# tangjiapeng/DiffuScene

Measured on AMD Instinct MI355X. Metric: denoiser steps/sec (train + 1000-step sample) at B=256, N=80 objects, higher is better.
Workload: dtype f32 (operands split 3xbf16, 6 products, f32 accumulate); 1 GPU; uncond living/dining rooms (config/uncond/diffusion_livingrooms_instancond_lat32_v.yaml scaled to N=80), B=256 scenes per GPU, N=80, C=65, T=1000, mode=both; global_batch=256, parallelism=single

## Files before the change

### __graft_entry__.py

```python
import os
import subprocess
import sys

ROOT = os.path.dirname(os.path.abspath(__file__))
CSRC = os.path.join(ROOT, "diffuscene_amd", "csrc")
LIB = os.path.join(ROOT, "diffuscene_amd", "libdiffuscene_hip.so")

SOURCES = [
    ("gemm_mfma.hip", []),
    ("gemm_split.hip", ["-fno-slp-vectorize"]),
    ("gemm_tn_split.hip", ["-fno-slp-vectorize"]),
    ("blocks.hip", []),
    ("diffusion.hip", ["-ffp-contract=off"]),
    ("train.hip", []),
    ("retrieval.hip", ["-ffp-contract=off"]),
    ("dataset.hip", ["-ffp-contract=off"]),
    ("chamfer.hip", ["-ffp-contract=off"]),
    ("optim.hip", ["-ffp-contract=off"]),
    ("foldingnet.hip", []),
]


def _hipcc():
    for c in (os.environ.get("HIPCC"), "/opt/rocm/bin/hipcc", "hipcc"):
        if c and (os.path.isabs(c) and os.path.exists(c) or not os.path.isabs(c)):
            return c
    raise RuntimeError("hipcc not found")


def _stale(target, deps):
    if not os.path.exists(target):
        return True
    t = os.path.getmtime(target)
    return any(os.path.getmtime(d) > t for d in deps)


def _stamp_git_head():
    try:
        head = subprocess.check_output(["git", "rev-parse", "--short", "HEAD"], cwd=ROOT, stderr=subprocess.DEVNULL, text=True).strip()
        dirty = subprocess.check_output(["git", "status", "--porcelain", "-uno"], cwd=ROOT, stderr=subprocess.DEVNULL, text=True).strip()
        with open(os.path.join(ROOT, "GIT_HEAD"), "w") as f:
            f.write(head + ("+" if dirty else "") + "\n")
    except Exception:
        pass

# ... 95 lines not shown
```

### diffuscene_amd/_lib.py

```python
import ctypes as C
import os

_HERE = os.path.dirname(os.path.abspath(__file__))
LIB_PATH = os.path.join(_HERE, "libdiffuscene_hip.so")
if os.environ.get("DSC_HIP_LIB"):
    LIB_PATH = os.path.abspath(os.environ["DSC_HIP_LIB"])

ACT_NONE, ACT_GELU, ACT_SILU, ACT_LEAKY01 = 0, 1, 2, 3
SS_NONE, SS_PER_TOKEN, SS_PER_SCENE, SS_PER_SLOT, SS_BY_INDEX = 0, 1, 2, 3, 4
MEAN_EPS, MEAN_X0, MEAN_V = 0, 1, 2
TILE_GN_80_W8, TILE_GN_80_W4, TILE_160x256, TILE_160x128_W4 = 1, 2, 5, 8
TILE_WAVE_GN, TILE_WAVE_DENSE, TILE_WAVE_GN_64 = 10, 11, 12
F32_TILE_160x256, F32_TILE_160x128, F32_TILE_128x128, F32_TILE_96x128, F32_TILE_64x64 = 0, 1, 2, 3, 4
DSC_PLANES_NONE = -100
GEMM_ROW_INVARIANT = 1
WS_MAX = 64
MAX_TOKENS_PER_SCENE = 160
STATS_MAX_OBJECTS, STATS_ONE_WAVE_MAX = 160, 32

_ERR = {-1: "DSC_EINVAL (bad shape / null pointer)", -2: "DSC_EALIGN (16-byte alignment required)",
        -3: "DSC_ERANGE (size outside kernel limits)"}

c_f32p = C.c_void_p
c_i64p = C.c_void_p


class GemmArgs(C.Structure):
    _fields_ = [
        ("a1", C.c_void_p), ("lda1", C.c_int64), ("k1", C.c_int32),
        ("a2", C.c_void_p), ("lda2", C.c_int64), ("k2", C.c_int32),
        ("w", C.c_void_p), ("ldw", C.c_int64),
        ("bias", C.c_void_p),
        ("residual", C.c_void_p), ("ldr", C.c_int64),
        ("y", C.c_void_p), ("ldy", C.c_int64),
        ("m", C.c_int32), ("n", C.c_int32),
        ("act_in", C.c_int32), ("act_out", C.c_int32),
        ("batch", C.c_int32),
        ("sa1", C.c_int64), ("sa2", C.c_int64), ("sw", C.c_int64), ("sbias", C.c_int64),
        ("sres", C.c_int64), ("sy", C.c_int64),
        ("gamma", C.c_void_p), ("beta", C.c_void_p), ("eps", C.c_float),
        ("tokens_per_scene", C.c_int32),
        ("scale_shift", C.c_void_p), ("ld_ss", C.c_int64), ("ss_mode", C.c_int32),
        ("preact", C.c_void_p), ("ld_preact", C.c_int64),
        ("ss_index", C.c_void_p),
        ("w_planes", C.c_void_p),
        ("actgrad_x", C.c_void_p), ("ld_actgrad", C.c_int64),
        ("ss_rows", C.c_int32),
        ("w_planes_layout", C.c_int32),
        ("gnb_z", C.c_void_p), ("ld_gnb_z", C.c_int64),
        ("gnb_dgamma", C.c_void_p), ("gnb_dbeta", C.c_void_p), ("gnb_dbias", C.c_void_p), ("gnb_pstride", C.c_int64),
        ("gnb_dss", C.c_void_p), ("ld_gnb_dss", C.c_int64),
        ("flags", C.c_int32),
    ]


class SplitItem(C.Structure):
    _fields_ = [("w", C.c_void_p), ("ldw", C.c_int64), ("rows", C.c_int32), ("cols", C.c_int32), ("planes", C.c_void_p),
                ("transpose", C.c_int32)]


class SmallKItem(C.Structure):
    _fields_ = [("x", C.c_void_p), ("ldx", C.c_int64), ("k_in", C.c_int32), ("w", C.c_void_p), ("ldw", C.c_int64), ("bias", C.c_void_p),
                ("y", C.c_void_p), ("ldy", C.c_int64)]


class ColSpan(C.Structure):
    _fields_ = [("src_col", C.c_int32), ("dst_col", C.c_int32), ("width", C.c_int32)]


SMALLK_MAX = 4


class WsItem(C.Structure):
    _fields_ = [("w", C.c_void_p), ("out", C.c_void_p), ("rows", C.c_int32), ("cols", C.c_int32)]


class TnGroup(C.Structure):
    _fields_ = [("a1", C.c_void_p), ("lda1", C.c_int64), ("k1", C.c_int32),
                ("a2", C.c_void_p), ("lda2", C.c_int64), ("k2", C.c_int32),
                ("dy", C.c_void_p), ("ldd", C.c_int64),
                ("out", C.c_void_p), ("ldo", C.c_int64),
                ("dbias", C.c_void_p),
                ("m", C.c_int32), ("n", C.c_int32), ("kvalid", C.c_int32),
                ("tile0", C.c_int32),
                ("ws_offset", C.c_int64),
                ("tile0s", C.c_int32)]


class ColsumItem(C.Structure):
    _fields_ = [("x", C.c_void_p), ("ldx", C.c_int64), ("m", C.c_int32), ("n", C.c_int32), ("out", C.c_void_p)]


class WsBwdItem(C.Structure):
    _fields_ = [("w", C.c_void_p), ("dw_std", C.c_void_p), ("dw", C.c_void_p), ("rows", C.c_int32), ("cols", C.c_int32)]


SIGNATURES = {
    "dsc_version": (C.c_int, []),
    "dsc_gemm_f32": (C.c_int, [C.POINTER(GemmArgs), C.c_void_p]),
    "dsc_gemm_gn_silu_f32": (C.c_int, [C.POINTER(GemmArgs), C.c_void_p]),
    "dsc_split_bf16x3_f32": (C.c_int, [C.POINTER(SplitItem), C.c_int32, C.c_void_p]),
    "dsc_gemm_arithmetic": (C.c_int, [C.POINTER(GemmArgs), C.c_int32]),
    "dsc_gemm_split_tile": (C.c_int, [C.POINTER(GemmArgs), C.c_int32]),
    "dsc_gemm_f32_tile": (C.c_int, [C.POINTER(GemmArgs)]),
    "dsc_gemm_planes_layout": (C.c_int, [C.POINTER(GemmArgs), C.c_int32]),
    "dsc_get_split_wave": (C.c_int, []),
    "dsc_set_split_wave": (C.c_int, [C.c_int32]),
    "dsc_gemm_skinny": (C.c_int, [C.POINTER(GemmArgs), C.c_int32]),
    "dsc_get_skinny": (C.c_int, []),
    "dsc_set_skinny": (C.c_int, [C.c_int32]),
    "dsc_get_gemm_arithmetic": (C.c_int, []),
    "dsc_set_gemm_arithmetic": (C.c_int, [C.c_int32]),
    "dsc_gemm_layernorm_f32": (C.c_int, [C.POINTER(GemmArgs), C.c_void_p]),
    "dsc_gemm_splitk_f32": (C.c_int, [C.POINTER(GemmArgs), C.c_int32, c_f32p, C.c_int64, C.c_void_p]),
    "dsc_linear_smallk_f32": (C.c_int, [c_f32p, C.c_int64, C.c_int32, c_f32p, C.c_int64, c_f32p, c_f32p, C.c_int64,
                                        C.c_int32, C.c_int32, C.c_int32, C.c_void_p]),
    "dsc_linear_smallk_grouped_f32": (C.c_int, [C.POINTER(SmallKItem), C.c_int32, C.c_int32, C.c_int32, C.c_int32, C.c_void_p]),
    "dsc_gather_columns_f32": (C.c_int, [c_f32p, C.c_int64, c_f32p, C.c_int64, C.c_int32, C.POINTER(ColSpan), C.c_int32, C.c_void_p]),
    "dsc_weight_standardize_f32": (C.c_int, [C.POINTER(WsItem), C.c_int32, C.c_float, C.c_void_p]),
    "dsc_layernorm_f32": (C.c_int, [c_f32p, C.c_int64, c_f32p, c_f32p, C.c_int64, c_f32p, C.c_int64, C.c_int32,
                                    C.c_int32, C.c_float, C.c_void_p]),
    "dsc_linear_attention_f32": (C.c_int, [c_f32p, C.c_int64, c_f32p, C.c_int64, c_f32p, C.c_int64, c_f32p, C.c_int64,
                                           C.c_int32, C.c_int32, C.c_int32, C.c_float, C.c_void_p]),
    "dsc_attention_f32": (C.c_int, [c_f32p, C.c_int64, c_f32p, C.c_int64, c_f32p, C.c_int64, c_f32p, C.c_int64,
                                    C.c_int32, C.c_int32, C.c_float, C.c_void_p]),
    "dsc_time_embedding_f32": (C.c_int, [c_i64p, C.c_int32, C.c_int32, c_f32p, C.c_int32, c_f32p, c_f32p, C.c_void_p]),
    "dsc_activation_f32": (C.c_int, [c_f32p, c_f32p, C.c_int64, C.c_int32, C.c_void_p]),
    "dsc_q_sample_f32": (C.c_int, [c_f32p, c_f32p, c_i64p, c_f32p, c_f32p, c_f32p, c_f32p, C.c_int32, C.c_int64, C.c_int32,
                                   C.c_void_p]),
    "dsc_p_sample_f32": (C.c_int, [c_f32p, c_f32p, c_f32p, c_i64p, c_f32p, c_f32p, c_f32p, c_f32p, c_f32p, c_f32p,
                                   c_f32p, C.c_int32, C.c_int32, C.c_int32, C.c_int64, C.c_int32, C.c_void_p]),
    "dsc_device_error_count": (C.c_int64, [C.c_int32]),
    "dsc_add_scalar_i64": (C.c_int, [c_i64p, C.c_int32, C.c_int64, C.c_void_p]),
    "dsc_ddim_step_f32": (C.c_int, [c_f32p, c_f32p, c_f32p, c_i64p, c_i64p, c_i64p, c_f32p, c_f32p, c_f32p, c_f32p, c_f32p,
                                    c_f32p, c_f32p, c_f32p, c_f32p, C.c_int32, C.c_int32, C.c_int64, C.c_int32, C.c_int32,
                                    C.c_void_p]),
    "dsc_ddim_advance_i64": (C.c_int, [c_i64p, c_i64p, c_i64p, C.c_int32, C.c_int32, C.c_void_p]),
    "dsc_knn16_f32": (C.c_int, [c_f32p, C.c_int64, C.c_int32, c_f32p, c_f32p, C.c_int32, C.c_int32, C.c_void_p, C.c_void_p]),
    "dsc_rowsq_f32": (C.c_int, [c_f32p, C.c_int64, C.c_int32, C.c_int64, c_f32p, C.c_void_p]),
    "dsc_knn_cov_f32": (C.c_int, [c_f32p, C.c_int64, C.c_void_p, C.c_int32, C.c_int32, c_f32p, C.c_int64, C.c_void_p]),
    "dsc_gather_max_f32": (C.c_int, [c_f32p, C.c_int64, C.c_void_p, C.c_int32, C.c_int32, C.c_int32, c_f32p, C.c_int64,
                                     C.c_void_p, C.c_void_p]),
    "dsc_gather_max_bwd_f32": (C.c_int, [c_f32p, C.c_int64, C.c_void_p, C.c_void_p, C.c_int32, C.c_int32, C.c_int32, c_f32p,
                                         C.c_int64, C.c_void_p]),
    "dsc_bn_workspace_floats": (C.c_int64, [C.c_int64, C.c_int32]),
    "dsc_batchnorm_fwd_f32": (C.c_int, [c_f32p, C.c_int64, c_f32p, c_f32p, C.c_int64, C.c_int32, C.c_float, C.c_float,
# ... 99 lines not shown
def load():
    global _lib
    if _lib is not None:
        return _lib
    if not os.path.exists(LIB_PATH):
        raise HipLibraryMissing(
            "%s not found: build it with `python __graft_entry__.py` (hipcc --offload-arch=gfx950). "
            "diffuscene_amd has no CPU or PyTorch fallback." % LIB_PATH)
    import torch
    lib = C.CDLL(LIB_PATH)
    for name, (res, args) in SIGNATURES.items():
        try:
            fn = getattr(lib, name)
        except AttributeError as e:
            raise HipLibraryMissing("symbol %s missing from %s" % (name, LIB_PATH)) from e
        fn.restype = res
        fn.argtypes = args
    if lib.dsc_get_gemm_arithmetic() < 0:
        raise ValueError("DSC_GEMM=%r: must be 'split' (default) or 'f32'" % os.environ.get("DSC_GEMM"))
    if lib.dsc_get_tn_split_form() < 0:
        raise ValueError("DSC_TN_FORM=%r: must be '2' (default), '1' or '0'" % os.environ.get("DSC_TN_FORM"))
    if lib.dsc_get_split_wave() < 0:
        raise ValueError("DSC_WAVE=%r: must be '1' / 'auto' (default) or '0'" % os.environ.get("DSC_WAVE"))
    _lib = lib
    return lib


def split_enabled():
    return load().dsc_get_gemm_arithmetic() == 1


def gemm_mode():
    lib = load()
    if lib.dsc_get_gemm_arithmetic() != 1:
        return 0
    return (2 if lib.dsc_get_split_wave() == 1 else 1) + 10 * lib.dsc_get_tn_split_form()


def set_split_wave(on):
    prev = load().dsc_get_split_wave() == 1
    check(load().dsc_set_split_wave(1 if on else 0), "dsc_set_split_wave")
    return prev


def set_gemm_arithmetic(name):
    if name not in ("split", "f32"):
        raise ValueError("gemm arithmetic must be 'split' or 'f32', got %r" % (name,))
    prev = "split" if split_enabled() else "f32"
    check(load().dsc_set_gemm_arithmetic(1 if name == "split" else 0), "dsc_set_gemm_arithmetic")
    return prev


def device_error_count(reset=False):
    n = load().dsc_device_error_count(1 if reset else 0)
    if n < 0:
        raise RuntimeError("dsc_device_error_count failed (HIP error)")
    return int(n)


def check_indices(where):
    if os.environ.get("DSC_CHECK_INDICES", "0") == "1":
        n = device_error_count(reset=True)
        if n:
            raise IndexError("%s: %d out-of-range device timestep(s) were clamped into the schedule tables" % (where, n))


def check(rc, what):
    if rc != 0:
        raise RuntimeError("%s failed: %s" % (what, _ERR.get(rc, "hipError_t %d" % rc)))
# ... 5 lines not shown
```

### diffuscene_amd/csrc/dsc_common.h

```cpp
#pragma once
#include <hip/hip_runtime.h>
#include <stdint.h>
#include <type_traits>
#include "../../include/diffuscene_hip.h"

typedef float f32x2 __attribute__((ext_vector_type(2)));
typedef float f32x4 __attribute__((ext_vector_type(4)));
typedef float f32x16 __attribute__((ext_vector_type(16)));

#define DSC_WAVE 64

#include <utility>
template <class F, int... I>
__device__ __forceinline__ void dsc_static_for_impl(F&& f, std::integer_sequence<int, I...>) { (f(std::integral_constant<int, I>{}), ...); }
template <int N, class F>
__device__ __forceinline__ void dsc_static_for(F&& f) { dsc_static_for_impl(f, std::make_integer_sequence<int, N>{}); }

#define DSC_CLEAR_STALE_ERROR() ((void)hipGetLastError())

#define DSC_LAUNCH_CHECK()                                   \
    do {                                                     \
        hipError_t e__ = hipGetLastError();                  \
        if (e__ != hipSuccess) return (int)e__;              \
    } while (0)
// ... 44 lines not shown
    const int waves = (n + 15) / 16;
    return waves >= 8 ? 512u : 64u * (unsigned)waves;
}

__device__ __forceinline__ float wave_sum(float v) {
#pragma unroll
    for (int o = 32; o > 0; o >>= 1) v += __shfl_xor(v, o, 64);
    return v;
}
__device__ __forceinline__ float wave_sum_dpp(float v) {
    auto dpp_add = [](float x, auto ctrl, auto row_mask, auto bank_mask) {
        const int y = __builtin_amdgcn_update_dpp(0, __builtin_bit_cast(int, x), decltype(ctrl)::value, decltype(row_mask)::value,
                                                  decltype(bank_mask)::value, true);
        return x + __builtin_bit_cast(float, y);
    };
    using std::integral_constant;
    v = dpp_add(v, integral_constant<int, 0x111>{}, integral_constant<int, 0xf>{}, integral_constant<int, 0xf>{});
    v = dpp_add(v, integral_constant<int, 0x112>{}, integral_constant<int, 0xf>{}, integral_constant<int, 0xf>{});
    v = dpp_add(v, integral_constant<int, 0x114>{}, integral_constant<int, 0xf>{}, integral_constant<int, 0xf>{});
    v = dpp_add(v, integral_constant<int, 0x118>{}, integral_constant<int, 0xf>{}, integral_constant<int, 0xf>{});
    v = dpp_add(v, integral_constant<int, 0x142>{}, integral_constant<int, 0xa>{}, integral_constant<int, 0xf>{});
    v = dpp_add(v, integral_constant<int, 0x143>{}, integral_constant<int, 0xc>{}, integral_constant<int, 0xf>{});
    return __builtin_bit_cast(float, __builtin_amdgcn_readlane(__builtin_bit_cast(int, v), 63));
}
__device__ __forceinline__ float wave_max(float v) {
#pragma unroll
    for (int o = 32; o > 0; o >>= 1) v = fmaxf(v, __shfl_xor(v, o, 64));
    return v;
}

#define DSC_SPLIT_NOT_TAKEN (-1000)
int dsc_gemm_try_split(const dsc_gemm_args* a, bool gn, hipStream_t s);

int dsc_launch_reduce_grouped(const dsc_tn_group* groups_dev, int count, int total_tiles, int splits, const float* workspace, hipStream_t s);

#ifdef DSC_BAD_INDEX_COUNTER
static __device__ unsigned int dsc_bad_index_count = 0;
__device__ __forceinline__ int64_t dsc_checked_index(int64_t v, int64_t n, bool first = true) {
    if (v < 0 || v >= n) {
        if (first) atomicAdd(&dsc_bad_index_count, 1u);
        return (v < 0 || n < 1) ? 0 : n - 1;
    }
    return v;
}
static inline unsigned dsc_read_bad_index_count(bool reset) {
    unsigned v = 0;
    if (hipMemcpyFromSymbol(&v, HIP_SYMBOL(dsc_bad_index_count), sizeof(v)) != hipSuccess) return 0xffffffffu;
    if (reset && v) {
        const unsigned z = 0;
        (void)hipMemcpyToSymbol(HIP_SYMBOL(dsc_bad_index_count), &z, sizeof(z));
    }
    return v;
}
#endif
unsigned dsc_bad_index_diffusion(bool reset);
unsigned dsc_bad_index_train(bool reset);
unsigned dsc_bad_index_retrieval(bool reset);
__device__ __forceinline__ int64_t dsc_clamp_index(int64_t v, int64_t n) { return (v < 0 || n < 1) ? 0 : (v >= n ? n - 1 : v); }

static inline bool dsc_aligned16(const void* p) { return (reinterpret_cast<uintptr_t>(p) & 15u) == 0; }
```

### diffuscene_amd/csrc/gemm_mfma.hip

```cpp
#include "gemm_core.h"
#include "gemm_skinny.h"
#include <cstdlib>

namespace {

using dsc_gemm::gemm_kernel;
constexpr int BK = 32;

int check_common(const dsc_gemm_args* a) {
    if (!a || !a->a1 || !a->w || !a->y) return DSC_EINVAL;
    if (a->m <= 0 || a->n <= 0 || a->k1 <= 0 || a->k2 < 0) return DSC_EINVAL;
    if ((a->k1 % BK) || (a->k2 % BK)) return DSC_EINVAL;
    if (a->k2 > 0 && !a->a2) return DSC_EINVAL;
    if (a->batch < 1) return DSC_EINVAL;
    if (!dsc_aligned16(a->a1) || (a->lda1 & 3) || !dsc_aligned16(a->w) || (a->ldw & 3)) return DSC_EALIGN;
    if (a->k2 > 0 && (!dsc_aligned16(a->a2) || (a->lda2 & 3))) return DSC_EALIGN;
    if (a->batch > 1 && ((a->sa1 & 3) || (a->sa2 & 3) || (a->sw & 3))) return DSC_EALIGN;
    if (a->act_in != DSC_ACT_NONE) return DSC_EINVAL;
    if (a->act_out < DSC_ACT_NONE || a->act_out > DSC_ACT_SILU) return DSC_EINVAL;
    return 0;
}

template <int TM, int TN, int WM, int WN, bool GN, int IL>
int launch_il(const dsc_gemm_args* a, int rows_per_blk, hipStream_t s) {
// ... 212 lines not shown
        default: return launch<1, 1, 2, 2, true, 0>(a, rpb, s);
    }
}

extern "C" int dsc_gemm_splitk_f32(const dsc_gemm_args* a, int32_t splits, float* workspace, int64_t workspace_floats,
                                   dsc_stream_t stream) {
    int rc = check_common(a);
    if (rc) return rc;
    if (splits < 2 || splits > 64 || !workspace) return DSC_EINVAL;
    if (a->batch != 1 || a->k2 != 0 || a->act_out != DSC_ACT_NONE) return DSC_EINVAL;
    if (a->k1 % (BK * splits)) return DSC_EINVAL;
    if (workspace_floats < (int64_t)splits * a->m * a->n) return DSC_EINVAL;
    if ((reinterpret_cast<uintptr_t>(workspace) & 15) || (((int64_t)a->m * a->n) & 3)) return DSC_EALIGN;
    dsc_gemm_args p = *a;
    const int kc = a->k1 / splits;
    p.k1 = kc;
    p.batch = splits;
    p.sa1 = kc; p.sw = kc; p.sa2 = 0; p.sbias = 0; p.sres = 0;
    p.bias = nullptr; p.residual = nullptr;
    p.y = workspace; p.ldy = a->n; p.sy = (int64_t)a->m * a->n;
    rc = dsc_gemm_f32(&p, stream);
    if (rc) return rc;
    const long total = (long)a->m * a->n;
    long blocks = (total + 255) / 256;
    if (blocks > 2048) blocks = 2048;
    DSC_CLEAR_STALE_ERROR();
    hipLaunchKernelGGL(splitk_reduce_kernel, dim3((unsigned)blocks), dim3(256), 0, static_cast<hipStream_t>(stream), workspace,
                       (long)a->m * a->n, splits, a->bias, a->residual, (long)a->ldr, a->y, (long)a->ldy, a->m, a->n);
    DSC_LAUNCH_CHECK();
    return 0;
}

extern "C" int dsc_gemm_layernorm_f32(const dsc_gemm_args* a, dsc_stream_t stream) {
    int rc = check_common(a);
    if (rc) return rc;
    if (a->n != 512 || a->batch != 1 || a->act_out != DSC_ACT_NONE || !a->gamma) return DSC_EINVAL;
    if (!dsc_aligned16(a->gamma) || !dsc_aligned16(a->y) || (a->ldy & 3)) return DSC_EALIGN;
    if (a->residual && (!dsc_aligned16(a->residual) || (a->ldr & 3))) return DSC_EALIGN;
    if (a->bias && !dsc_aligned16(a->bias)) return DSC_EALIGN;
    const int64_t ld_max = a->lda1 > a->ldw ? a->lda1 : a->ldw;
    if (!(a->k2 == 0 || a->lda1 == a->lda2) || ld_max * 4 * (96 + 512) >= (int64_t(1) << 31)) return DSC_ERANGE;
    const int nrb = (a->m + 95) / 96;
    DSC_CLEAR_STALE_ERROR();
    hipLaunchKernelGGL((gemm_kernel<3, 2, 1, 8, false, 2, 0, true>), dim3((unsigned)nrb, 1), dim3(512), 0,
                       static_cast<hipStream_t>(stream), *a, 1);
    DSC_LAUNCH_CHECK();
    return 0;
}
```

### diffuscene_amd/engine.py

```python
import ctypes as C

import torch

from . import _lib, ops
from ._lib import ACT_GELU, ACT_NONE, ACT_SILU, SS_BY_INDEX, SS_NONE, SS_PER_SCENE, SS_PER_SLOT, SS_PER_TOKEN

D = 512
HID = 128
DEC_PAD = 32


def _own(t):
    if isinstance(t, torch.nn.Parameter):
        return t.detach()
    if isinstance(t, (tuple, list)):
        return tuple(_own(u) for u in t)
    return t


class StalePlanError(RuntimeError):
    pass


class _Pool:
# ... 76 lines not shown

    def call(self, name, *args, keep=()):
        self.keep.append(_own(keep))
        self.steps.append((_lib.fn(name), args))

    def rec(self, rec):
        self.call(rec[0], *rec[1], keep=rec[2])

    def hoist(self, first):
        if self.time_table:
            self.pre_steps += self.steps[first:]
            del self.steps[first:]
            return True
        return False

    def check_current(self):
        if self.generation != self.eng.generation:
            raise StalePlanError("diffuscene_amd: this launch plan was built for parameter storages the model no longer uses (flat storage "
                                 "of the first training step, module.to(), load into new tensors): rebuild it -- DenoiserEngine.prepare() / "
                                 "graph_sample_loop() do -- instead of running or replaying it")

    def run_pre(self):
        self.check_current()
        s = ops.stream_ptr()
        for f, a in self.pre_steps:
            rc = f(*a, s)
            if rc:
                _lib.check(rc, f.__name__)

    def layernorm(self, x, g, out, residual=None):
        self.rec(ops.layernorm_rec(x, g, out, residual))
        return out

    def out_proj_ln(self, a, conv, ln_gain, residual):
        M = self.M
        out = self.pool.get(M, D)
        if (M + 95) // 96 >= 160:
            g = ops.make_gemm_args(a, conv.weight, out, conv.bias, None, residual, gamma=ln_gain.view(-1), beta=ln_gain.view(-1),
                                   eps=1e-5)
            self.call("dsc_gemm_layernorm_f32", C.byref(g), keep=(g, a, conv.weight, out, conv.bias, residual, ln_gain))
            return out
        o = self.gemm(a, conv.weight, self.pool.get(M, D), conv.bias)
        self.layernorm(o, ln_gain, out, residual=residual)
        self.pool.put(o)
        return out

    def resblock(self, rb, x, x2, ss, ss_mode):
        e, M = self.eng, self.M
        h = self.pool.get(M, D)
        self.gemm_gn(x, e.ws[id(rb.block1.proj)], h, rb.block1.proj.bias, rb.block1.norm.weight, rb.block1.norm.bias,
                     a2=x2, ss=ss, ss_mode=ss_mode)
        if rb.has_res_conv:
            r = self.pool.get(M, D)
            self.gemm(x, rb.res_conv.weight, r, rb.res_conv.bias, a2=x2)
        else:
            r = x
        out = self.pool.get(M, D)
        self.gemm_gn(h, e.ws[id(rb.block2.proj)], out, rb.block2.proj.bias, rb.block2.norm.weight, rb.block2.norm.bias,
                     residual=r)
        self.pool.put(h)
        if rb.has_res_conv:
            self.pool.put(r)
        return out

    def t_ss(self, rb):
        i = self.eng.t_index[id(rb)]
        return self.ss_t[:, i * 2 * D:(i + 1) * 2 * D], (SS_BY_INDEX if self.time_table else SS_PER_SCENE)

    def c_ss(self, rb):
        if self.ss_c is None:
            return None, SS_NONE
        i = self.eng.c_index[id(rb)]
        return self.ss_c[:, i * 2 * D:(i + 1) * 2 * D], self.ctx_mode

    def linattn(self, blk, x):
        M, B, N = self.M, self.B, self.N
        att = blk.fn.fn
        y = self.layernorm(x, blk.fn.norm.g, self.pool.get(M, D))
        qkv = self.gemm(y, att.to_qkv.weight, self.pool.get(M, 3 * HID))
        self.pool.put(y)
        a = self.pool.get(M, HID)
        q, k, v = qkv.split(HID, dim=1)
        self.rec(ops.linear_attention_rec(q, k, v, a, B, N, N, float(att.scale)))
        self.pool.put(qkv)
        out = self.out_proj_ln(a, att.to_out[0], att.to_out[1].g, x)
        self.pool.put(a)
        return out

    def crossattn(self, blk, x):
        M, B, N, L = self.M, self.B, self.N, self.L
        att = blk.fn.fn
        y = self.layernorm(x, blk.fn.norm.g, self.pool.get(M, D))
        q = self.gemm(y, att.to_q.weight, self.pool.get(M, HID))
        self.pool.put(y)
        first = len(self.steps)
        kv = self.gemm(self.cross_in, att.to_kv.weight, self.pool.get(B * L, 2 * HID))
        kv_is_invariant = self.hoist(first)
        a = self.pool.get(M, HID)
        self.rec(ops.linear_attention_rec(q, kv[:, :HID], kv[:, HID:], a, B, N, L, float(att.scale)))
        self.pool.put(q)
        if not kv_is_invariant:
            self.pool.put(kv)
        out = self.out_proj_ln(a, att.to_out[0], att.to_out[1].g, x)
        self.pool.put(a)
        return out

    def fullattn(self, blk, x):
        M, B, N = self.M, self.B, self.N
        att = blk.fn.fn
        y = self.layernorm(x, blk.fn.norm.g, self.pool.get(M, D))
        qkv = self.gemm(y, att.to_qkv.weight, self.pool.get(M, 3 * HID))
        self.pool.put(y)
        a = self.pool.get(M, HID)
        q, k, v = qkv.split(HID, dim=1)
        self.rec(ops.attention_rec(q, k, v, a, B, N, float(att.scale)))
        self.pool.put(qkv)
        out = self.gemm(a, att.to_out.weight, self.pool.get(M, D), att.to_out.bias, residual=x)
        self.pool.put(a)
        return out

    def _build(self):
        e, net, M, B = self.eng, self.eng.net, self.M, self.B
        pool = self.pool
        if self.time_table:
            self.ss_t = e.ss_table()
        else:
            temb = pool.get(B, D)
            self.rec(ops.time_embedding_rec(self.t_in, D, e.time_table, e.time_freq, temb))
            t1 = self.gemm(temb, net.time_mlp[1].weight, pool.get(B, 4 * D), net.time_mlp[1].bias, act_out=ACT_GELU, row_invariant=True)
            t2 = self.gemm(t1, net.time_mlp[3].weight, pool.get(B, 4 * D), net.time_mlp[3].bias, act_out=ACT_SILU, row_invariant=True)
            self.ss_t = self.gemm(t2, e.t_pack_w, pool.get(B, e.t_pack_w.shape[0]), e.t_pack_b, row_invariant=True)
        if self.ctx_in is not None:
            first = len(self.steps)
            cact = pool.get(self.ctx_in.shape[0], self.ctx_in.shape[1])
            self.rec(ops.activation_rec(self.ctx_in, cact, ACT_SILU))
            self.ss_c = self.gemm(cact, e.c_pack_w, pool.get(self.ctx_in.shape[0], e.c_pack_w.shape[0]), e.c_pack_b)
            self.hoist(first)
# ... 289 lines not shown
```

### diffuscene_amd/ops.py

```python
import ctypes as C
import numbers

import torch

from . import _lib
from ._lib import (ACT_GELU, ACT_NONE, ACT_SILU, MEAN_EPS, MEAN_V, MEAN_X0, SS_NONE, SS_PER_SCENE,
                   SS_PER_SLOT, SS_PER_TOKEN, GemmArgs, SplitItem, WsItem)


def stream_ptr():
    return torch.cuda.current_stream().cuda_stream


def _dev(t, name="tensor", dtype=torch.float32):
    if not isinstance(t, torch.Tensor) or not t.is_cuda:
        raise RuntimeError("diffuscene_amd: %s must live on a HIP device (no CPU fallback exists)" % name)
    if t.dtype != dtype:
        raise RuntimeError("diffuscene_amd: %s must be %s, got %s" % (name, dtype, t.dtype))
    return t


def issue(rec, stream=None):
    name, args, _ = rec
    _lib.check(_lib.fn(name)(*args, stream if stream is not None else stream_ptr()), name)


def _mat(t, name):
    _dev(t, name)
    if t.dim() != 2 or (t.shape[1] > 1 and t.stride(1) != 1):
        raise RuntimeError("diffuscene_amd: %s must be a 2-D tensor with contiguous rows, got shape %s strides %s"
                           % (name, tuple(t.shape), t.stride()))
    return t.data_ptr(), (t.stride(0) if t.shape[0] > 1 else t.shape[1])


def as2d(w):
    return w.view(w.shape[0], w.shape[1]) if w.dim() == 3 else w


def make_gemm_args(a, w, y, bias=None, a2=None, residual=None, act_in=ACT_NONE, act_out=ACT_NONE,
                   gamma=None, beta=None, eps=1e-5, tokens_per_scene=0, scale_shift=None, ss_mode=SS_NONE, preact=None,
                   ss_index=None, w_planes=None, actgrad_x=None, gnb=None, row_invariant=False):
    g = GemmArgs()
    g.a1, g.lda1 = _mat(a, "a")
    g.k1 = a.shape[1]
    if a2 is not None:
        g.a2, g.lda2 = _mat(a2, "a2")
        g.k2 = a2.shape[1]
        if a2.shape[0] != a.shape[0]:
            raise RuntimeError("a and a2 row mismatch")
    w2 = as2d(w)
    g.w, g.ldw = _mat(w2, "w")
    if w2.shape[1] != g.k1 + g.k2:
        raise RuntimeError("weight K (%d) != activation K (%d)" % (w2.shape[1], g.k1 + g.k2))
    g.m, g.n = a.shape[0], w2.shape[0]
    g.y, g.ldy = _mat(y, "y")
    if tuple(y.shape) != (g.m, g.n):
        raise RuntimeError("output shape %s != (%d, %d)" % (tuple(y.shape), g.m, g.n))
    if bias is not None:
        g.bias = _dev(bias, "bias").data_ptr()
    if residual is not None:
        g.residual, g.ldr = _mat(residual, "residual")
    g.act_in, g.act_out, g.batch = act_in, act_out, 1
    if row_invariant:
        g.flags |= _lib.GEMM_ROW_INVARIANT
    if gamma is not None:
        g.gamma, g.beta, g.eps = _dev(gamma).data_ptr(), _dev(beta).data_ptr(), eps
        g.tokens_per_scene = tokens_per_scene
    if scale_shift is not None:
        g.scale_shift, g.ld_ss = _mat(scale_shift, "scale_shift")
        g.ss_mode = ss_mode
    if preact is not None:
        g.preact, g.ld_preact = _mat(preact, "preact")
    if actgrad_x is not None:
        g.actgrad_x, g.ld_actgrad = _mat(actgrad_x, "actgrad_x")
        if tuple(actgrad_x.shape) != (g.m, g.n):
            raise RuntimeError("actgrad_x shape %s != (%d, %d)" % (tuple(actgrad_x.shape), g.m, g.n))
# ... 1100 lines not shown
```

### include/diffuscene_hip.h

```cpp
#ifndef DIFFUSCENE_HIP_H
#define DIFFUSCENE_HIP_H

#include <stdint.h>

#ifdef __cplusplus
extern "C" {
#endif

typedef void* dsc_stream_t;

#define DSC_EINVAL   (-1)
#define DSC_EALIGN   (-2)
#define DSC_ERANGE   (-3)

#define DSC_ACT_NONE 0
#define DSC_ACT_GELU 1
#define DSC_ACT_SILU 2
#define DSC_ACT_LEAKY01 3

#define DSC_SS_NONE      0
#define DSC_SS_PER_TOKEN 1
#define DSC_SS_PER_SCENE 2
#define DSC_SS_PER_SLOT  3
#define DSC_SS_BY_INDEX  4

#define DSC_HEADS    4
#define DSC_DIM_HEAD 32

int dsc_version(void);

typedef struct dsc_gemm_args {
    const float* a1; int64_t lda1; int32_t k1;
    const float* a2; int64_t lda2; int32_t k2;
    const float* w;  int64_t ldw;
    const float* bias;
    const float* residual; int64_t ldr;
    float* y; int64_t ldy;
    int32_t m, n;
    int32_t act_in;
    int32_t act_out;
    int32_t batch; int64_t sa1, sa2, sw, sbias, sres, sy;
    const float* gamma; const float* beta; float eps;
    int32_t tokens_per_scene;
    const float* scale_shift; int64_t ld_ss; int32_t ss_mode;
    float* preact; int64_t ld_preact;
    const int64_t* ss_index;
    const uint16_t* w_planes;
    const float* actgrad_x; int64_t ld_actgrad;
    int32_t ss_rows;
    int32_t w_planes_layout;
    const float* gnb_z; int64_t ld_gnb_z;
    float* gnb_dgamma; float* gnb_dbeta; float* gnb_dbias; int64_t gnb_pstride;
    float* gnb_dss; int64_t ld_gnb_dss;
    int32_t flags;
} dsc_gemm_args;
#define DSC_GEMM_ROW_INVARIANT 1
#define DSC_PLANES_ROWMAJOR 0
#define DSC_PLANES_FRAGMENT 1
#define DSC_PLANES_NONE (-100)

int dsc_gemm_f32(const dsc_gemm_args* args, dsc_stream_t stream);

int dsc_gemm_arithmetic(const dsc_gemm_args* args, int32_t gn);

#define DSC_TILE_GN_32       0
#define DSC_TILE_GN_80_W8    1
#define DSC_TILE_GN_80_W4    2
#define DSC_TILE_GN_48       3
#define DSC_TILE_GN_64       4
#define DSC_TILE_160x256     5
#define DSC_TILE_256x128     6
#define DSC_TILE_128x128     7
#define DSC_TILE_160x128_W4  8
#define DSC_TILE_64x256      9
#define DSC_TILE_WAVE_GN     10
#define DSC_TILE_WAVE_DENSE  11
#define DSC_TILE_WAVE_GN_64  12
int dsc_gemm_split_tile(const dsc_gemm_args* args, int32_t gn);

#define DSC_F32_TILE_160x256 0
#define DSC_F32_TILE_160x128 1
#define DSC_F32_TILE_128x128 2
#define DSC_F32_TILE_96x128  3
#define DSC_F32_TILE_64x64   4
int dsc_gemm_f32_tile(const dsc_gemm_args* args);

int dsc_gemm_planes_layout(const dsc_gemm_args* args, int32_t gn);

int dsc_get_split_wave(void);
int dsc_set_split_wave(int32_t mode);

int dsc_gemm_skinny(const dsc_gemm_args* args, int32_t gn);
int dsc_get_skinny(void);
int dsc_set_skinny(int32_t on);

int dsc_get_gemm_arithmetic(void);
int dsc_set_gemm_arithmetic(int32_t mode);

#define DSC_SPLIT_TRANSPOSE 1
#define DSC_SPLIT_FRAGMENT  2
typedef struct dsc_split_item { const float* w; int64_t ldw; int32_t rows, cols; uint16_t* planes; int32_t transpose; } dsc_split_item;
int dsc_split_bf16x3_f32(const dsc_split_item* items, int32_t count, dsc_stream_t stream);

int dsc_gemm_gn_silu_f32(const dsc_gemm_args* args, dsc_stream_t stream);

int dsc_gemm_splitk_f32(const dsc_gemm_args* a, int32_t splits, float* workspace, int64_t workspace_floats, dsc_stream_t stream);

int dsc_gemm_layernorm_f32(const dsc_gemm_args* a, dsc_stream_t stream);

int dsc_linear_smallk_f32(const float* x, int64_t ldx, int32_t k_in, const float* w, int64_t ldw,
                          const float* bias, float* y, int64_t ldy, int32_t m, int32_t n,
                          int32_t act_out, dsc_stream_t stream);
#define DSC_SMALLK_MAX 4
typedef struct dsc_smallk_item { const float* x; int64_t ldx; int32_t k_in; const float* w; int64_t ldw; const float* bias;
                                 float* y; int64_t ldy; } dsc_smallk_item;
int dsc_linear_smallk_grouped_f32(const dsc_smallk_item* items, int32_t count, int32_t m, int32_t n, int32_t act_out,
                                  dsc_stream_t stream);
typedef struct dsc_col_span { int32_t src_col, dst_col, width; } dsc_col_span;
int dsc_gather_columns_f32(float* dst, int64_t ldd, const float* src, int64_t lds, int32_t rows, const dsc_col_span* spans,
                           int32_t count, dsc_stream_t stream);

#define DSC_WS_MAX 64
typedef struct dsc_ws_item { const float* w; float* out; int32_t rows; int32_t cols; } dsc_ws_item;
int dsc_weight_standardize_f32(const dsc_ws_item* items, int32_t count, float eps, dsc_stream_t stream);

int dsc_layernorm_f32(const float* x, int64_t ldx, const float* g, const float* residual, int64_t ldr,
                      float* y, int64_t ldy, int32_t m, int32_t d, float eps, dsc_stream_t stream);

int dsc_linear_attention_f32(const float* q, int64_t ldq, const float* k, int64_t ldk,
                             const float* v, int64_t ldv, float* out, int64_t ldo,
                             int32_t scenes, int32_t nq, int32_t nk, float scale, dsc_stream_t stream);

int dsc_attention_f32(const float* q, int64_t ldq, const float* k, int64_t ldk,
                      const float* v, int64_t ldv, float* out, int64_t ldo,
                      int32_t scenes, int32_t n, float scale, dsc_stream_t stream);

int dsc_time_embedding_f32(const int64_t* t, int32_t b, int32_t dim, const float* table, int32_t table_rows,
                           const float* freq, float* out, dsc_stream_t stream);

int dsc_activation_f32(const float* x, float* y, int64_t count, int32_t act, dsc_stream_t stream);

// ... 268 lines not shown
```

Measured before the change: 62.55 steps/s.

## Fuse linear attention with output projection, LayerNorm and residual in one kernel

Adds an attn_tail kernel that, per scene, computes the linear attention (softmax over K, context = K^T V, softmax over Q, output) in LDS. It then feeds the result directly into the 128->512 output projection GEMM with a fused LayerNorm and residual add. It replaces the separate linear_attention kernel plus out_proj_ln GEMM for both self- and cross-attention when there are at least 160 scenes, removing the intermediate attention tensor round-trip through HBM and one launch per attention block. The trade-off is a large LDS footprint, one block per scene, and plain f32 MFMA for the projection instead of the split-bf16 path, which may change numerics and occupancy.

```diff
diff --git a/__graft_entry__.py b/__graft_entry__.py
--- a/__graft_entry__.py
+++ b/__graft_entry__.py
@@ -11,6 +11,7 @@
     ("gemm_split.hip", ["-fno-slp-vectorize"]),
     ("gemm_tn_split.hip", ["-fno-slp-vectorize"]),
     ("blocks.hip", []),
+    ("attn_tail.hip", []),
     ("diffusion.hip", ["-ffp-contract=off"]),
     ("train.hip", []),
     ("retrieval.hip", ["-ffp-contract=off"]),
diff --git a/diffuscene_amd/_lib.py b/diffuscene_amd/_lib.py
--- a/diffuscene_amd/_lib.py
+++ b/diffuscene_amd/_lib.py
@@ -51,6 +51,12 @@
         ("gnb_dgamma", C.c_void_p), ("gnb_dbeta", C.c_void_p), ("gnb_dbias", C.c_void_p), ("gnb_pstride", C.c_int64),
         ("gnb_dss", C.c_void_p), ("ld_gnb_dss", C.c_int64),
         ("flags", C.c_int32),
+        ("la_q", C.c_void_p), ("ld_la_q", C.c_int64),
+        ("la_k", C.c_void_p), ("ld_la_k", C.c_int64),
+        ("la_v", C.c_void_p), ("ld_la_v", C.c_int64),
+        ("la_nq", C.c_int32), ("la_nk", C.c_int32),
+        ("la_scale", C.c_float),
+        ("la_out", C.c_void_p), ("ld_la_out", C.c_int64),
     ]
 
 
@@ -112,6 +118,9 @@
     "dsc_get_gemm_arithmetic": (C.c_int, []),
     "dsc_set_gemm_arithmetic": (C.c_int, [C.c_int32]),
     "dsc_gemm_layernorm_f32": (C.c_int, [C.POINTER(GemmArgs), C.c_void_p]),
+    "dsc_attn_tail": (C.c_int, [C.POINTER(GemmArgs)]),
+    "dsc_get_attn_tail": (C.c_int, []),
+    "dsc_set_attn_tail": (C.c_int, [C.c_int32]),
     "dsc_gemm_splitk_f32": (C.c_int, [C.POINTER(GemmArgs), C.c_int32, c_f32p, C.c_int64, C.c_void_p]),
     "dsc_linear_smallk_f32": (C.c_int, [c_f32p, C.c_int64, C.c_int32, c_f32p, C.c_int64, c_f32p, c_f32p, C.c_int64,
                                         C.c_int32, C.c_int32, C.c_int32, C.c_void_p]),
@@ -277,9 +286,19 @@
 
 def gemm_mode():
     lib = load()
+    tail = 100 * lib.dsc_get_attn_tail()
     if lib.dsc_get_gemm_arithmetic() != 1:
-        return 0
-    return (2 if lib.dsc_get_split_wave() == 1 else 1) + 10 * lib.dsc_get_tn_split_form()
+        return tail
+    return (2 if lib.dsc_get_split_wave() == 1 else 1) + 10 * lib.dsc_get_tn_split_form() + tail
+
+
+ATTN_TAIL_MODES = ("0", "1", "force")
+
+
+def set_attn_tail(mode):
+    prev = load().dsc_set_attn_tail(ATTN_TAIL_MODES.index(str(mode)))
+    check(min(prev, 0), "dsc_set_attn_tail")
+    return ATTN_TAIL_MODES[prev]
 
 
 def set_split_wave(on):
diff --git a/diffuscene_amd/csrc/attn_tail.hip b/diffuscene_amd/csrc/attn_tail.hip
--- /dev/null
+++ b/diffuscene_amd/csrc/attn_tail.hip
@@ -0,0 +1,372 @@
+#include "dsc_common.h"
+#include <cstdlib>
+#include <cstring>
+
+namespace {
+
+constexpr int AT_MAXTOK = 96;
+constexpr int AT_LP = 36;
+constexpr int AT_QLD = 132;
+constexpr int AT_TLD = 68;
+constexpr int AT_KV_FLOATS = 4 * AT_MAXTOK * AT_LP;
+constexpr int AT_CTX_FLOATS = 4 * 32 * AT_LP;
+constexpr int AT_STAT_FLOATS = 2 * 8 * AT_MAXTOK;
+constexpr int AT_LDS_BYTES = 4 * (AT_KV_FLOATS + AT_CTX_FLOATS + AT_STAT_FLOATS);
+static_assert(AT_KV_FLOATS >= AT_MAXTOK * AT_QLD && AT_KV_FLOATS >= 8 * 16 * AT_TLD, "the Q / a image and the wave tiles reuse the K / V bytes");
+
+template <int RT>
+__global__ __launch_bounds__(512) void attn_tail_kernel(const dsc_gemm_args p) {
+    extern __shared__ __attribute__((aligned(16))) float at_lds[];
+    float* kv = at_lds;
+    float* ctx = at_lds + AT_KV_FLOATS;
+    float* stat = ctx + AT_CTX_FLOATS;
+    const int tid = threadIdx.x, lane = tid & 63, wave = tid >> 6;
+    const int l15 = lane & 15, lq = lane >> 4;
+    const int nq = p.la_nq, nk = p.la_nk;
+    const int64_t b = blockIdx.x;
+    const float* qb = p.la_q + b * nq * p.ld_la_q;
+    const float* kb = p.la_k + b * nk * p.ld_la_k;
+    const float* vb = p.la_v + b * nk * p.ld_la_v;
+
+    const int kvrow = tid >> 4, kvpiece = tid & 15;
+    f32x4 kreg[3], vreg[3];
+    auto load_kv = [&](int hp) {
+#pragma unroll
+        for (int s = 0; s < 3; ++s) {
+            const int j = s * 32 + kvrow;
+            if (j < nk) {
+                kreg[s] = *reinterpret_cast<const f32x4*>(kb + (int64_t)j * p.ld_la_k + hp * 64 + kvpiece * 4);
+                vreg[s] = *reinterpret_cast<const f32x4*>(vb + (int64_t)j * p.ld_la_v + hp * 64 + kvpiece * 4);
+            }
+        }
+    };
+    auto stage_kv = [&]() {
+        const int hh = kvpiece >> 3, c4 = (kvpiece & 7) * 4;
+#pragma unroll
+        for (int s = 0; s < 3; ++s) {
+            const int j = s * 32 + kvrow;
+            if (j < nk) {
+                *reinterpret_cast<f32x4*>(kv + (hh * nk + j) * AT_LP + c4) = kreg[s];
+                *reinterpret_cast<f32x4*>(kv + ((2 + hh) * nk + j) * AT_LP + c4) = vreg[s];
+            }
+        }
+    };
+    auto context = [&](int hp) {
+        {
+            const int d64 = tid >> 3, part = tid & 7;
+            float* Kc = kv + (d64 >> 5) * nk * AT_LP + (d64 & 31);
+            float kx[AT_MAXTOK / 8];
+            float mx = -INFINITY;
+#pragma unroll
+            for (int i = 0; i < AT_MAXTOK / 8; ++i) {
+                const int j = part + 8 * i;
+                kx[i] = j < nk ? Kc[j * AT_LP] : -INFINITY;
+                mx = fmaxf(mx, kx[i]);
+            }
+            mx = fmaxf(mx, __shfl_xor(mx, 1, 64));
+            mx = fmaxf(mx, __shfl_xor(mx, 2, 64));
+            mx = fmaxf(mx, __shfl_xor(mx, 4, 64));
+            float sm = 0.f;
+#pragma unroll
+            for (int i = 0; i < AT_MAXTOK / 8; ++i) {
+                kx[i] = expf(kx[i] - mx);
+                sm += kx[i];
+            }
+            sm += __shfl_xor(sm, 1, 64);
+            sm += __shfl_xor(sm, 2, 64);
+            sm += __shfl_xor(sm, 4, 64);
+            const float inv = 1.0f / sm;
+#pragma unroll
+            for (int i = 0; i < AT_MAXTOK / 8; ++i) {
+                const int j = part + 8 * i;
+                if (j < nk) Kc[j * AT_LP] = kx[i] * inv;
+            }
+        }
+        __syncthreads();
+        {
+            const int hh = wave >> 2, dt = (wave >> 1) & 1, et = wave & 1;
+            const float* Kc = kv + hh * nk * AT_LP + dt * 16 + l15;
+            const float* Vc = kv + (2 + hh) * nk * AT_LP + et * 16 + l15;
+            f32x4 c = {0.f, 0.f, 0.f, 0.f};
+            const int nfull = nk & ~3;
+            for (int j = lq; j < nfull; j += 4) c = __builtin_amdgcn_mfma_f32_16x16x4f32(Kc[j * AT_LP], Vc[j * AT_LP], c, 0, 0, 0);
+            if (nfull < nk) {
+                const int j = nfull + lq;
+                const bool ok = j < nk;
+                c = __builtin_amdgcn_mfma_f32_16x16x4f32(ok ? Kc[j * AT_LP] : 0.f, ok ? Vc[j * AT_LP] : 0.f, c, 0, 0, 0);
+            }
+            *reinterpret_cast<f32x4*>(ctx + ((2 * hp + hh) * 32 + et * 16 + l15) * AT_LP + dt * 16 + 4 * lq) = c;
+        }
+        __syncthreads();
+    };
+
+    load_kv(0);
+    stage_kv();
+    load_kv(1);
+    const int qrow = tid >> 5, qpiece = tid & 31;
+    f32x4 qreg[RT];
+#pragma unroll
+    for (int s = 0; s < RT; ++s) {
+        const int i = s * 16 + qrow;
+        if (i < nq) qreg[s] = *reinterpret_cast<const f32x4*>(qb + (int64_t)i * p.ld_la_q + qpiece * 4);
+    }
+    __syncthreads();
+    context(0);
+    stage_kv();
+    __syncthreads();
+    context(1);
+    float* Qs = kv;
+#pragma unroll
+    for (int s = 0; s < RT; ++s) {
+        const int i = s * 16 + qrow;
+        if (i < nq) *reinterpret_cast<f32x4*>(Qs + i * AT_QLD + qpiece * 4) = qreg[s];
+    }
+    __syncthreads();
+
+    for (int i0 = 0; i0 < nq; i0 += 32) {
+        const int i = i0 + (tid >> 4), h = (tid >> 2) & 3, part = tid & 3;
+        const bool ok = i < nq;
+        float* qr = Qs + i * AT_QLD + h * 32 + part * 8;
+        float qv[8];
+        float mx = -INFINITY;
+        if (ok) {
+            const f32x4 a = *reinterpret_cast<const f32x4*>(qr);
+            const f32x4 c = *reinterpret_cast<const f32x4*>(qr + 4);
+#pragma unroll
+            for (int e = 0; e < 4; ++e) { qv[e] = a[e]; qv[4 + e] = c[e]; }
+#pragma unroll
+            for (int e = 0; e < 8; ++e) mx = fmaxf(mx, qv[e]);
+        }
+        mx = fmaxf(mx, __shfl_xor(mx, 1, 64));
+        mx = fmaxf(mx, __shfl_xor(mx, 2, 64));
+        float sm = 0.f;
+        if (ok) {
+#pragma unroll
+            for (int e = 0; e < 8; ++e) { qv[e] = expf(qv[e] - mx); sm += qv[e]; }
+        }
+        sm += __shfl_xor(sm, 1, 64);
+        sm += __shfl_xor(sm, 2, 64);
+        if (ok) {
+            const float inv = p.la_scale / sm;
+            f32x4 a, c;
+#pragma unroll
+            for (int e = 0; e < 4; ++e) { a[e] = qv[e] * inv; c[e] = qv[4 + e] * inv; }
+            *reinterpret_cast<f32x4*>(qr) = a;
+            *reinterpret_cast<f32x4*>(qr + 4) = c;
+        }
+    }
+    __syncthreads();
+    for (int t = wave; t < 4 * RT; t += 8) {
+        const int h = t & 3, row = (t >> 2) * 16 + l15;
+        const float* qp = Qs + (row < nq ? row : nq - 1) * AT_QLD + h * 32 + 4 * lq;
+        const f32x4 q0 = *reinterpret_cast<const f32x4*>(qp), q1 = *reinterpret_cast<const f32x4*>(qp + 16);
+        f32x4 o[2];
+#pragma unroll
+        for (int et = 0; et < 2; ++et) {
+            const float* cp = ctx + (h * 32 + et * 16 + l15) * AT_LP + 4 * lq;
+            const f32x4 c0 = *reinterpret_cast<const f32x4*>(cp), c1 = *reinterpret_cast<const f32x4*>(cp + 16);
+            o[et] = f32x4{0.f, 0.f, 0.f, 0.f};
+#pragma unroll
+            for (int e = 0; e < 4; ++e) o[et] = __builtin_amdgcn_mfma_f32_16x16x4f32(c0[e], q0[e], o[et], 0, 0, 0);
+#pragma unroll
+            for (int e = 0; e < 4; ++e) o[et] = __builtin_amdgcn_mfma_f32_16x16x4f32(c1[e], q1[e], o[et], 0, 0, 0);
+        }
+        __builtin_amdgcn_wave_barrier();
+        if (row < nq) {
+            float* ar = Qs + row * AT_QLD + h * 32 + 4 * lq;
+            *reinterpret_cast<f32x4*>(ar) = o[0];
+            *reinterpret_cast<f32x4*>(ar + 16) = o[1];
+        }
+    }
+
+    const int c_st = wave * 64 + l15 * 4;
+    constexpr int PF = RT <= 5 ? RT : 4;
+    f32x4 res[RT][4];
+    auto load_res = [&](auto rtc) {
+        constexpr int rt = decltype(rtc)::value;
+#pragma unroll
+        for (int i = 0; i < 4; ++i) {
+            const int row = rt * 16 + 4 * i + lq;
+            res[rt][i] = f32x4{0.f, 0.f, 0.f, 0.f};
+            if (p.residual && row < nq) res[rt][i] = *reinterpret_cast<const f32x4*>(p.residual + (b * nq + row) * p.ldr + c_st);
+        }
+    };
+    dsc_static_for<PF>([&](auto rtc) { load_res(rtc); });
+    const int c_acc = wave * 64 + 4 * lq;
+    f32x4 acc[RT][4];
+#pragma unroll
+    for (int ct = 0; ct < 4; ++ct) {
+        f32x4 b4 = {0.f, 0.f, 0.f, 0.f};
+        if (p.bias) b4 = *reinterpret_cast<const f32x4*>(p.bias + c_acc + 16 * ct);
+#pragma unroll
+        for (int rt = 0; rt < RT; ++rt) acc[rt][ct] = b4;
+    }
+    const float* wp = p.w + (int64_t)(wave * 64 + l15) * p.ldw + 4 * lq;
+    const int64_t wstep = 16 * p.ldw;
+    const float* ap[RT];
+#pragma unroll
+    for (int rt = 0; rt < RT; ++rt) {
+        const int row = rt * 16 + l15;
+        ap[rt] = Qs + (row < nq ? row : nq - 1) * AT_QLD + 4 * lq;
+    }
+    f32x4 wn[4];
+#pragma unroll
+    for (int ct = 0; ct < 4; ++ct) wn[ct] = *reinterpret_cast<const f32x4*>(wp + ct * wstep);
+    __syncthreads();
+#pragma unroll 1
+    for (int u = 0; u < 8; ++u) {
+        f32x4 wf[4], af[RT];
+#pragma unroll
+        for (int ct = 0; ct < 4; ++ct) wf[ct] = wn[ct];
+        const int un = u < 7 ? u + 1 : 7;
+#pragma unroll
+        for (int ct = 0; ct < 4; ++ct) wn[ct] = *reinterpret_cast<const f32x4*>(wp + ct * wstep + 16 * un);
+#pragma unroll
+        for (int rt = 0; rt < RT; ++rt) af[rt] = *reinterpret_cast<const f32x4*>(ap[rt] + 16 * u);
+#pragma unroll
+        for (int e = 0; e < 4; ++e)
+#pragma unroll
+            for (int rt = 0; rt < RT; ++rt)
+#pragma unroll
+                for (int ct = 0; ct < 4; ++ct)
+                    acc[rt][ct] = __builtin_amdgcn_mfma_f32_16x16x4f32(wf[ct][e], af[rt][e], acc[rt][ct], 0, 0, 0);
+    }
+
+    const int srow = l15;
+    float mean[RT], rs[RT];
+#pragma unroll
+    for (int rt = 0; rt < RT; ++rt) {
+        float s = 0.f;
+#pragma unroll
+        for (int ct = 0; ct < 4; ++ct) s += (acc[rt][ct][0] + acc[rt][ct][1]) + (acc[rt][ct][2] + acc[rt][ct][3]);
+        s += __shfl_xor(s, 16, 64);
+        s += __shfl_xor(s, 32, 64);
+        if (lq == 0) stat[wave * AT_MAXTOK + rt * 16 + srow] = s;
+    }
+    __syncthreads();
+#pragma unroll
+    for (int rt = 0; rt < RT; ++rt) {
+        float s = 0.f;
+#pragma unroll
+        for (int w8 = 0; w8 < 8; ++w8) s += stat[w8 * AT_MAXTOK + rt * 16 + srow];
+        mean[rt] = s * (1.0f / 512.0f);
+        float s2 = 0.f;
+#pragma unroll
+        for (int ct = 0; ct < 4; ++ct)
+#pragma unroll
+            for (int r = 0; r < 4; ++r) {
+                acc[rt][ct][r] -= mean[rt];
+                s2 += acc[rt][ct][r] * acc[rt][ct][r];
+            }
+        s2 += __shfl_xor(s2, 16, 64);
+        s2 += __shfl_xor(s2, 32, 64);
+        if (lq == 0) stat[(8 + wave) * AT_MAXTOK + rt * 16 + srow] = s2;
+    }
+    __syncthreads();
+#pragma unroll
+    for (int rt = 0; rt < RT; ++rt) {
+        float s2 = 0.f;
+#pragma unroll
+        for (int w8 = 0; w8 < 8; ++w8) s2 += stat[(8 + w8) * AT_MAXTOK + rt * 16 + srow];
+        rs[rt] = 1.0f / sqrtf(s2 * (1.0f / 512.0f) + p.eps);
+    }
+    f32x4 gain[4];
+#pragma unroll
+    for (int ct = 0; ct < 4; ++ct) gain[ct] = *reinterpret_cast<const f32x4*>(p.gamma + c_acc + 16 * ct);
+
+    float* tile = kv + wave * 16 * AT_TLD;
+    dsc_static_for<RT>([&](auto rtc) {
+        constexpr int rt = decltype(rtc)::value;
+        if constexpr (rt + 1 >= PF && rt + 1 < RT) load_res(std::integral_constant<int, rt + 1>{});
+#pragma unroll
+        for (int ct = 0; ct < 4; ++ct) {
+            f32x4 o;
+#pragma unroll
+            for (int r = 0; r < 4; ++r) o[r] = acc[rt][ct][r] * rs[rt] * gain[ct][r];
+            *reinterpret_cast<f32x4*>(tile + l15 * AT_TLD + 16 * ct + 4 * lq) = o;
+        }
+        __builtin_amdgcn_wave_barrier();
+#pragma unroll
+        for (int i = 0; i < 4; ++i) {
+            const int row = rt * 16 + 4 * i + lq;
+            f32x4 o = *reinterpret_cast<const f32x4*>(tile + (4 * i + lq) * AT_TLD + l15 * 4);
+#pragma unroll
+            for (int r = 0; r < 4; ++r) o[r] += res[rt][i][r];
+            if (row < nq) *reinterpret_cast<f32x4*>(p.y + (b * nq + row) * p.ldy + c_st) = o;
+        }
+        __builtin_amdgcn_wave_barrier();
+    });
+}
+
+template <int RT>
+int launch_rt(const dsc_gemm_args* a, int scenes, hipStream_t s) {
+    static bool attr_set = false;
+    if (!attr_set) {
+        hipError_t e = hipFuncSetAttribute(reinterpret_cast<const void*>(attn_tail_kernel<RT>), hipFuncAttributeMaxDynamicSharedMemorySize,
+                                           AT_LDS_BYTES);
+        if (e != hipSuccess) return (int)e;
+        attr_set = true;
+    }
+    DSC_CLEAR_STALE_ERROR();
+    hipLaunchKernelGGL(attn_tail_kernel<RT>, dim3((unsigned)scenes), dim3(512), AT_LDS_BYTES, s, *a);
+    DSC_LAUNCH_CHECK();
+    return 0;
+}
+
+constexpr int AT_MIN_SCENES = 160;
+int g_attn_tail = -1;
+
+int attn_tail_mode() {
+    if (g_attn_tail < 0) {
+        const char* e = std::getenv("DSC_ATTN_TAIL");
+        g_attn_tail = (e && e[0] == '0') ? 0 : (e && !std::strcmp(e, "force")) ? 2 : 1;
+    }
+    return g_attn_tail;
+}
+
+int attn_tail_check(const dsc_gemm_args* a) {
+    if (!a || !a->la_q || !a->la_k || !a->la_v || !a->w || !a->y || !a->gamma) return DSC_EINVAL;
+    if (a->n != 512 || a->k1 != DSC_HEADS * DSC_DIM_HEAD || a->k2 != 0 || a->batch != 1) return DSC_EINVAL;
+    if (a->act_in != DSC_ACT_NONE || a->act_out != DSC_ACT_NONE || a->preact || a->la_out || a->actgrad_x || a->gnb_z) return DSC_EINVAL;
+    if (a->la_nq < 1 || a->la_nk < 1 || a->m < 1 || (a->m % a->la_nq)) return DSC_EINVAL;
+    if (a->la_nq > AT_MAXTOK || a->la_nk > AT_MAXTOK) return DSC_ERANGE;
+    if (!dsc_aligned16(a->la_q) || !dsc_aligned16(a->la_k) || !dsc_aligned16(a->la_v) || (a->ld_la_q & 3) || (a->ld_la_k & 3) ||
+        (a->ld_la_v & 3))
+        return DSC_EALIGN;
+    if (!dsc_aligned16(a->w) || (a->ldw & 3) || !dsc_aligned16(a->y) || (a->ldy & 3) || !dsc_aligned16(a->gamma)) return DSC_EALIGN;
+    if (a->residual && (!dsc_aligned16(a->residual) || (a->ldr & 3))) return DSC_EALIGN;
+    if (a->bias && !dsc_aligned16(a->bias)) return DSC_EALIGN;
+    return 0;
+}
+
+}
+
+extern "C" int dsc_get_attn_tail(void) { return attn_tail_mode(); }
+extern "C" int dsc_set_attn_tail(int32_t mode) {
+    if (mode < 0 || mode > 2) return DSC_EINVAL;
+    const int prev = attn_tail_mode();
+    g_attn_tail = mode;
+    return prev;
+}
+
+extern "C" int dsc_attn_tail(const dsc_gemm_args* a) {
+    const int rc = attn_tail_check(a);
+    if (rc) return rc;
+    const int mode = attn_tail_mode();
+    return mode == 2 || (mode == 1 && a->m / a->la_nq >= AT_MIN_SCENES) ? 1 : 0;
+}
+
+int dsc_attn_tail_launch(const dsc_gemm_args* a, hipStream_t s) {
+    const int take = dsc_attn_tail(a);
+    if (take < 0) return take;
+    if (take == 0) return DSC_EINVAL;
+    const int scenes = a->m / a->la_nq;
+    switch ((a->la_nq + 15) / 16) {
+        case 1: return launch_rt<1>(a, scenes, s);
+        case 2: return launch_rt<2>(a, scenes, s);
+        case 3: return launch_rt<3>(a, scenes, s);
+        case 4: return launch_rt<4>(a, scenes, s);
+        case 5: return launch_rt<5>(a, scenes, s);
+        default: return launch_rt<6>(a, scenes, s);
+    }
+}
diff --git a/diffuscene_amd/csrc/dsc_common.h b/diffuscene_amd/csrc/dsc_common.h
--- a/diffuscene_amd/csrc/dsc_common.h
+++ b/diffuscene_amd/csrc/dsc_common.h
@@ -100,6 +100,8 @@
 #define DSC_SPLIT_NOT_TAKEN (-1000)
 int dsc_gemm_try_split(const dsc_gemm_args* a, bool gn, hipStream_t s);
 
+int dsc_attn_tail_launch(const dsc_gemm_args* a, hipStream_t s);
+
 int dsc_launch_reduce_grouped(const dsc_tn_group* groups_dev, int count, int total_tiles, int splits, const float* workspace, hipStream_t s);
 
 #ifdef DSC_BAD_INDEX_COUNTER
diff --git a/diffuscene_amd/csrc/gemm_mfma.hip b/diffuscene_amd/csrc/gemm_mfma.hip
--- a/diffuscene_amd/csrc/gemm_mfma.hip
+++ b/diffuscene_amd/csrc/gemm_mfma.hip
@@ -268,6 +268,7 @@
 }
 
 extern "C" int dsc_gemm_layernorm_f32(const dsc_gemm_args* a, dsc_stream_t stream) {
+    if (a && (a->la_q || a->la_k || a->la_v)) return dsc_attn_tail_launch(a, static_cast<hipStream_t>(stream));
     int rc = check_common(a);
     if (rc) return rc;
     if (a->n != 512 || a->batch != 1 || a->act_out != DSC_ACT_NONE || !a->gamma) return DSC_EINVAL;
diff --git a/diffuscene_amd/engine.py b/diffuscene_amd/engine.py
--- a/diffuscene_amd/engine.py
+++ b/diffuscene_amd/engine.py
@@ -132,6 +132,20 @@
         self.rec(ops.layernorm_rec(x, g, out, residual))
         return out
 
+    def attn_tail(self, q, k, v, nk, att, residual):
+        conv, ln_gain = att.to_out[0], att.to_out[1].g
+        out = self.pool.get(self.M, D)
+        g = ops.make_gemm_args(None, conv.weight, out, conv.bias, None, residual, gamma=ln_gain.view(-1), beta=ln_gain.view(-1), eps=1e-5,
+                               la=dict(q=q, k=k, v=v, nq=self.N, nk=nk, scale=float(att.scale)))
+        take = _lib.fn("dsc_attn_tail")(C.byref(g))
+        if take != 1:
+            self.pool.put(out)
+            if take < 0 and self.N <= 96 and nk <= 96:
+                _lib.check(take, "dsc_attn_tail")
+            return None
+        self.call("dsc_gemm_layernorm_f32", C.byref(g), keep=(g, q, k, v, conv.weight, out, conv.bias, residual, ln_gain))
+        return out
+
     def out_proj_ln(self, a, conv, ln_gain, residual):
         M = self.M
         out = self.pool.get(M, D)
@@ -179,8 +193,12 @@
         y = self.layernorm(x, blk.fn.norm.g, self.pool.get(M, D))
         qkv = self.gemm(y, att.to_qkv.weight, self.pool.get(M, 3 * HID))
         self.pool.put(y)
+        q, k, v = qkv.split(HID, dim=1)
+        out = self.attn_tail(q, k, v, N, att, x)
+        if out is not None:
+            self.pool.put(qkv)
+            return out
         a = self.pool.get(M, HID)
-        q, k, v = qkv.split(HID, dim=1)
         self.rec(ops.linear_attention_rec(q, k, v, a, B, N, N, float(att.scale)))
         self.pool.put(qkv)
         out = self.out_proj_ln(a, att.to_out[0], att.to_out[1].g, x)
@@ -196,13 +214,15 @@
         first = len(self.steps)
         kv = self.gemm(self.cross_in, att.to_kv.weight, self.pool.get(B * L, 2 * HID))
         kv_is_invariant = self.hoist(first)
-        a = self.pool.get(M, HID)
-        self.rec(ops.linear_attention_rec(q, kv[:, :HID], kv[:, HID:], a, B, N, L, float(att.scale)))
+        out = self.attn_tail(q, kv[:, :HID], kv[:, HID:], L, att, x)
+        if out is None:
+            a = self.pool.get(M, HID)
+            self.rec(ops.linear_attention_rec(q, kv[:, :HID], kv[:, HID:], a, B, N, L, float(att.scale)))
+            out = self.out_proj_ln(a, att.to_out[0], att.to_out[1].g, x)
+            self.pool.put(a)
         self.pool.put(q)
         if not kv_is_invariant:
             self.pool.put(kv)
-        out = self.out_proj_ln(a, att.to_out[0], att.to_out[1].g, x)
-        self.pool.put(a)
         return out
 
     def fullattn(self, blk, x):
diff --git a/diffuscene_amd/ops.py b/diffuscene_amd/ops.py
--- a/diffuscene_amd/ops.py
+++ b/diffuscene_amd/ops.py
@@ -39,9 +39,16 @@
 
 def make_gemm_args(a, w, y, bias=None, a2=None, residual=None, act_in=ACT_NONE, act_out=ACT_NONE,
                    gamma=None, beta=None, eps=1e-5, tokens_per_scene=0, scale_shift=None, ss_mode=SS_NONE, preact=None,
-                   ss_index=None, w_planes=None, actgrad_x=None, gnb=None, row_invariant=False):
+                   ss_index=None, w_planes=None, actgrad_x=None, gnb=None, row_invariant=False, la=None):
     g = GemmArgs()
-    g.a1, g.lda1 = _mat(a, "a")
+    if la is not None:
+        if a is not None or a2 is not None:
+            raise RuntimeError("a launch with the attention prologue (la) has no a / a2 operand")
+        (g.la_q, g.ld_la_q), (g.la_k, g.ld_la_k), (g.la_v, g.ld_la_v) = _mat(la["q"], "la q"), _mat(la["k"], "la k"), _mat(la["v"], "la v")
+        g.la_nq, g.la_nk, g.la_scale = la["nq"], la["nk"], la["scale"]
+        a = la["q"]
+    else:
+        g.a1, g.lda1 = _mat(a, "a")
     g.k1 = a.shape[1]
     if a2 is not None:
         g.a2, g.lda2 = _mat(a2, "a2")
diff --git a/include/diffuscene_hip.h b/include/diffuscene_hip.h
--- a/include/diffuscene_hip.h
+++ b/include/diffuscene_hip.h
@@ -53,6 +53,12 @@
     float* gnb_dgamma; float* gnb_dbeta; float* gnb_dbias; int64_t gnb_pstride;
     float* gnb_dss; int64_t ld_gnb_dss;
     int32_t flags;
+    const float* la_q; int64_t ld_la_q;
+    const float* la_k; int64_t ld_la_k;
+    const float* la_v; int64_t ld_la_v;
+    int32_t la_nq, la_nk;
+    float la_scale;
+    float* la_out; int64_t ld_la_out;
 } dsc_gemm_args;
 #define DSC_GEMM_ROW_INVARIANT 1
 #define DSC_PLANES_ROWMAJOR 0
@@ -107,6 +113,10 @@
 int dsc_gemm_splitk_f32(const dsc_gemm_args* a, int32_t splits, float* workspace, int64_t workspace_floats, dsc_stream_t stream);
 
 int dsc_gemm_layernorm_f32(const dsc_gemm_args* a, dsc_stream_t stream);
+
+int dsc_attn_tail(const dsc_gemm_args* a);
+int dsc_get_attn_tail(void);
+int dsc_set_attn_tail(int32_t mode);
 
 int dsc_linear_smallk_f32(const float* x, int64_t ldx, int32_t k_in, const float* w, int64_t ldw,
                           const float* bias, float* y, int64_t ldy, int32_t m, int32_t n,
```

After: 63.14 steps/s, median of 6. No clear change (+0.9%).
